# HakimNessah/th_rl

Measured on AMD Instinct MI355X. Metric: env-steps/sec, 2-agent PD x 1M parallel games, higher is better.
Workload: dtype f32

## Files before the change

### th_rl_amd/csrc/thrl_wave_kernel.h

```cpp
#pragma once
#include <type_traits>
#include <utility>
#include "thrl_kernels.h"
#include "thrl_wave_lut.h"

#ifndef THRL_ABLATE
#define THRL_ABLATE 0
#endif

namespace thrl {

constexpr int kAblate = THRL_ABLATE;

typedef unsigned int v2u __attribute__((ext_vector_type(2)));

__device__ __forceinline__ v2u pack_halves(unsigned a, unsigned b) {
    return __builtin_amdgcn_permlane32_swap(a, b, false, false);
}

__device__ __forceinline__ unsigned lds_addr(const void* p) {
    return (unsigned)(uintptr_t)(__attribute__((address_space(3))) const void*)p;
}
template <typename QT>
__device__ __forceinline__ QT lds_load(unsigned addr) {
    typedef __attribute__((address_space(3))) QT lds_t;
    return *(const lds_t*)(uintptr_t)addr;
}
template <typename QT>
__device__ __forceinline__ void lds_store(unsigned addr, QT v) {
    typedef __attribute__((address_space(3))) QT lds_t;
    *(lds_t*)(uintptr_t)addr = v;
}

__device__ __forceinline__ void lds_inc(unsigned addr) {
    typedef unsigned __attribute__((may_alias)) u32_alias;
    typedef __attribute__((address_space(3))) u32_alias lds_u32;
    __hip_atomic_fetch_add((lds_u32*)(uintptr_t)addr, 1u, __ATOMIC_RELAXED, __HIP_MEMORY_SCOPE_WAVEFRONT);
}
__device__ __forceinline__ void lds_zero8(unsigned addr) {
    typedef unsigned long long __attribute__((may_alias)) u64_alias;
    typedef __attribute__((address_space(3))) u64_alias lds_u64;
    *(lds_u64*)(uintptr_t)addr = 0ull;
}

__device__ __forceinline__ unsigned bperm(unsigned byte_sel, unsigned v) {
    return (unsigned)__builtin_amdgcn_ds_bpermute((int)byte_sel, (int)v);
}

template <int CTRL>
__device__ __forceinline__ double dpp_mov64(double v) {
    const int lo = __double2loint(v), hi = __double2hiint(v);
    return __hiloint2double(__builtin_amdgcn_update_dpp(hi, hi, CTRL, 0xF, 0xF, false),
                            __builtin_amdgcn_update_dpp(lo, lo, CTRL, 0xF, 0xF, false));
}
template <int CTRL>
__device__ __forceinline__ uint32_t dpp_mov32(uint32_t v) {
    return (uint32_t)__builtin_amdgcn_update_dpp((int)v, (int)v, CTRL, 0xF, 0xF, false);
}

__device__ __forceinline__ float group8_allmax(float v) {
    asm("s_nop 1\n\t"
        "v_max_f32_dpp %0, %0, %0 quad_perm:[1,0,3,2] row_mask:0xf bank_mask:0xf\n\t"
        "s_nop 1\n\t"
        "v_max_f32_dpp %0, %0, %0 quad_perm:[2,3,0,1] row_mask:0xf bank_mask:0xf\n\t"
        "s_nop 1\n\t"
        "v_max_f32_dpp %0, %0, %0 row_half_mirror row_mask:0xf bank_mask:0xf"
        : "+v"(v));
    return v;
}
__device__ __forceinline__ double group8_allmax(double v) {
    v = fmax(v, dpp_mov64<0xB1>(v));
    v = fmax(v, dpp_mov64<0x4E>(v));
    v = fmax(v, dpp_mov64<0x141>(v));
    return v;
}
__device__ __forceinline__ void store_where(unsigned long long mask, unsigned addr, float v) {
    unsigned long long save;
    asm volatile("s_mov_b64 %0, exec\n\ts_mov_b64 exec, %1\n\tds_write_b32 %2, %3\n\ts_mov_b64 exec, %0"
                 : "=&s"(save) : "s"(mask), "v"(addr), "v"(v) : "memory");
}
__device__ __forceinline__ void store_where(unsigned long long mask, unsigned addr, double v) {
    unsigned long long save;
    asm volatile("s_mov_b64 %0, exec\n\ts_mov_b64 exec, %1\n\tds_write_b64 %2, %3\n\ts_mov_b64 exec, %0"
                 : "=&s"(save) : "s"(mask), "v"(addr), "v"(v) : "memory");
}
template <int IMM>
__device__ __forceinline__ void store_key(unsigned key, unsigned want, unsigned addr, float v) {
    if constexpr (IMM >= 0)
        asm volatile("v_cmpx_eq_u32 vcc, %0, %1\n\tds_write_b32 %2, %3\n\ts_mov_b64 exec, -1"
                     :: "n"(IMM), "v"(key), "v"(addr), "v"(v) : "memory", "vcc");
    else
        asm volatile("v_cmpx_eq_u32 vcc, %0, %1\n\tds_write_b32 %2, %3\n\ts_mov_b64 exec, -1"
                     :: "s"(want), "v"(key), "v"(addr), "v"(v) : "memory", "vcc");
}
template <int IMM>
__device__ __forceinline__ void store_key(unsigned key, unsigned want, unsigned addr, double v) {
    if constexpr (IMM >= 0)
        asm volatile("v_cmpx_eq_u32 vcc, %0, %1\n\tds_write_b64 %2, %3\n\ts_mov_b64 exec, -1"
                     :: "n"(IMM), "v"(key), "v"(addr), "v"(v) : "memory", "vcc");
    else
        asm volatile("v_cmpx_eq_u32 vcc, %0, %1\n\tds_write_b64 %2, %3\n\ts_mov_b64 exec, -1"
                     :: "s"(want), "v"(key), "v"(addr), "v"(v) : "memory", "vcc");
}
constexpr unsigned kKeyShift = 25;
constexpr unsigned kKeyNone = 0x7Fu;
__device__ __forceinline__ float dpp_ror8(float v) { return __builtin_bit_cast(float, dpp_mov32<0x128>(__builtin_bit_cast(uint32_t, v))); }
__device__ __forceinline__ double dpp_ror8(double v) { return dpp_mov64<0x128>(v); }
__device__ __forceinline__ float max_of(float a, float b) { return fmaxf(a, b); }
__device__ __forceinline__ double max_of(double a, double b);
__device__ __forceinline__ float half32_allmax(float v) {
    v = group8_allmax(v);
    v = fmaxf(v, __builtin_bit_cast(float, dpp_mov32<0x140>(__builtin_bit_cast(uint32_t, v))));
    unsigned a = __builtin_bit_cast(unsigned, v), b = a;
    asm("" : "+v"(b));
    const v2u r = __builtin_amdgcn_permlane16_swap(a, b, false, false);
    const unsigned rx = r.x, ry = r.y;
    return fmaxf(__builtin_bit_cast(float, rx), __builtin_bit_cast(float, ry));
}
__device__ __forceinline__ double half32_allmax(double v) {
    v = group8_allmax(v);
    v = fmax(v, dpp_mov64<0x140>(v));
    unsigned lo = (unsigned)__double2loint(v), hi = (unsigned)__double2hiint(v);
    unsigned lo2 = lo, hi2 = hi;
    asm("" : "+v"(lo2), "+v"(hi2));
    const v2u rl = __builtin_amdgcn_permlane16_swap(lo, lo2, false, false);
    const v2u rh = __builtin_amdgcn_permlane16_swap(hi, hi2, false, false);
    const unsigned rlx = rl.x, rly = rl.y, rhx = rh.x, rhy = rh.y;
    return fmax(__hiloint2double((int)rhx, (int)rlx), __hiloint2double((int)rhy, (int)rly));
}
__device__ __forceinline__ double max_of(double a, double b) { return fmax(a, b); }

__device__ __forceinline__ double wave_sum4(double q0, double q1, double q2, double q3, int lane) {
    const bool odd = lane & 1;
    const double k0 = odd ? q1 : q0, k1 = odd ? q3 : q2;
    const double s0 = odd ? q0 : q1, s1 = odd ? q2 : q3;
    const double a0 = k0 + dpp_mov64<0xB1>(s0);
    const double a1 = k1 + dpp_mov64<0xB1>(s1);
    const bool b1 = lane & 2;
    const double kk = b1 ? a1 : a0, ss = b1 ? a0 : a1;
    double v = kk + dpp_mov64<0x4E>(ss);
    v = v + dpp_mov64<0x124>(v);
    v = v + dpp_mov64<0x128>(v);
    {
        unsigned lo = (unsigned)__double2loint(v), hi = (unsigned)__double2hiint(v);
        unsigned lo2 = lo, hi2 = hi;
        asm("" : "+v"(lo2), "+v"(hi2));
        const v2u rl = __builtin_amdgcn_permlane16_swap(lo, lo2, false, false);
        const v2u rh = __builtin_amdgcn_permlane16_swap(hi, hi2, false, false);
        const unsigned rlx = rl.x, rly = rl.y, rhx = rh.x, rhy = rh.y;
        v = __hiloint2double((int)rhx, (int)rlx) + __hiloint2double((int)rhy, (int)rly);
    }
    {
        unsigned lo = (unsigned)__double2loint(v), hi = (unsigned)__double2hiint(v);
        unsigned lo2 = lo, hi2 = hi;
        asm("" : "+v"(lo2), "+v"(hi2));
        const v2u rl = __builtin_amdgcn_permlane32_swap(lo, lo2, false, false);
        const v2u rh = __builtin_amdgcn_permlane32_swap(hi, hi2, false, false);
        const unsigned rlx = rl.x, rly = rl.y, rhx = rh.x, rhy = rh.y;
        v = __hiloint2double((int)rhx, (int)rlx) + __hiloint2double((int)rhy, (int)rly);
    }
    return v;
}

template <int CTRL>
__device__ __forceinline__ uint32_t dpp_src(uint32_t v) {
    return (uint32_t)__builtin_amdgcn_update_dpp(0, (int)v, CTRL, 0xF, 0xF, true);
}

__device__ __forceinline__ float max3_f32(float a, float b, float c) {
    float r;
    asm("v_max3_f32 %0, %1, %2, %3" : "=v"(r) : "v"(a), "v"(b), "v"(c));
    return r;
}
__device__ __forceinline__ uint32_t argmax21_first(unsigned row) {
    float g[7];
#pragma unroll
    for (int k = 0; k < 7; k++)
        g[k] = max3_f32(lds_load<float>(row + 12u * k), lds_load<float>(row + 12u * k + 4u), lds_load<float>(row + 12u * k + 8u));
    const float m = max3_f32(max3_f32(g[0], g[1], g[2]), max3_f32(g[3], g[4], g[5]), g[6]);
    uint32_t c3 = 18u;
#pragma unroll
    for (int k = 5; k >= 0; k--) c3 = (g[k] == m) ? (uint32_t)(3 * k) : c3;
    const unsigned ad = row + 4u * c3;
    const float va = lds_load<float>(ad), vb = lds_load<float>(ad + 4u);
    uint32_t pos = (vb == m) ? 1u : 2u;
    pos = (va == m) ? 0u : pos;
    const float v0 = lds_load<float>(row);
    return (v0 != v0) ? 0u : c3 + pos;
}

__device__ __forceinline__ uint32_t readlane_u(uint32_t v, int lane) {
    return (uint32_t)__builtin_amdgcn_readlane((int)v, lane);
}

__device__ __forceinline__ uint32_t writelane_u(uint32_t old, uint32_t val, int lane) {
    asm("s_mov_b32 m0, %2\n\ts_nop 0\n\tv_writelane_b32 %0, %1, m0" : "+v"(old) : "s"(val), "s"(lane));
    return old;
}

__device__ __forceinline__ uint32_t halves_sum(uint32_t x) {
    uint32_t y;
    asm("v_add_u32_sdwa %0, %1, %1 dst_sel:DWORD dst_unused:UNUSED_PAD src0_sel:WORD_0 src1_sel:WORD_1" : "=v"(y) : "v"(x));
    return y;
}

template <int T0>
__device__ __forceinline__ void chain_group(uint32_t& sq, int& s, uint32_t n0, uint32_t n1, uint32_t n2, uint32_t n3) {
    int s1, s2, s3, s4, pk;
    asm volatile(
        "s_nop 3\n\t"
        "v_readlane_b32 %1, %7, %6\n\t"
        "s_pack_ll_b32_b16 %5, %6, %1\n\t"
        "v_writelane_b32 %0, %5, %11\n\t"
        "s_nop 1\n\t"
        "v_readlane_b32 %2, %8, %1\n\t"
        "s_nop 3\n\t"
        "v_readlane_b32 %3, %9, %2\n\t"
        "s_pack_ll_b32_b16 %5, %2, %3\n\t"
        "v_writelane_b32 %0, %5, %12\n\t"
        "s_nop 1\n\t"
        "v_readlane_b32 %4, %10, %3"
        : "+v"(sq), "=&s"(s1), "=&s"(s2), "=&s"(s3), "=&s"(s4), "=&s"(pk)
        : "s"(s), "v"(n0), "v"(n1), "v"(n2), "v"(n3), "n"(T0), "n"(T0 + 2)
        : "scc");
    s = s4;
}

template <int T0>
__device__ __forceinline__ void chain_group_greedy(uint32_t& sq, int& s, uint32_t g1, uint32_t g2, uint32_t g3, uint32_t g4) {
    int s1, s2, s3, s4, pk;
    asm volatile(
        "s_nop 3\n\t"
        "v_readlane_b32 %1, %7, %6\n\t"
        "v_readlane_b32 %2, %8, %6\n\t"
        "v_readlane_b32 %3, %9, %6\n\t"
        "v_readlane_b32 %4, %10, %6\n\t"
        "s_pack_ll_b32_b16 %5, %6, %1\n\t"
        "v_writelane_b32 %0, %5, %11\n\t"
        "s_pack_ll_b32_b16 %5, %2, %3\n\t"
        "v_writelane_b32 %0, %5, %12"
        : "+v"(sq), "=&s"(s1), "=&s"(s2), "=&s"(s3), "=&s"(s4), "=&s"(pk)
        : "s"(s), "v"(g1), "v"(g2), "v"(g3), "v"(g4), "n"(T0), "n"(T0 + 2)
        : "scc");
    s = s4;
}

template <bool ON> struct GreedyTables {
    __device__ __forceinline__ void build(unsigned) {}
    template <int T0> __device__ __forceinline__ void chain(uint32_t&, int&) const {}
};
template <> struct GreedyTables<true> {
    uint32_t g1, g2, g3, g4;
    __device__ __forceinline__ void build(unsigned lut_addr) {
        g1 = (uint32_t)lds_load<unsigned short>(lut_addr);
        g2 = bperm((g1 & 63u) << 2, g1);
        g3 = bperm((g2 & 63u) << 2, g1);
        g4 = bperm((g2 & 63u) << 2, g2);
    }
    template <int T0> __device__ __forceinline__ void chain(uint32_t& sq, int& s) const { chain_group_greedy<T0>(sq, s, g1, g2, g3, g4); }
};

template <int NRSEG>
__device__ __forceinline__ uint32_t read_row(const uint32_t (&r)[NRSEG], int s) {
    uint32_t v = readlane_u(r[0], s & 63);
    if (NRSEG > 1) {
        const uint32_t h = readlane_u(r[NRSEG - 1], s & 63);
        if (s >= 64) v = h;
    }
    return v;
}
template <int NRSEG>
__device__ __forceinline__ uint32_t gather_row(const uint32_t (&r)[NRSEG], uint32_t row) {
    uint32_t v = bperm((row & 63u) << 2, r[0]);
    if (NRSEG > 1) {
        const uint32_t h = bperm((row & 63u) << 2, r[NRSEG - 1]);
        if (row >= 64u) v = h;
    }
    return v;
}

template <typename QT> struct BlockOps;
template <> struct BlockOps<float> {
    unsigned c1;
    __device__ __forceinline__ void permute(unsigned sel) { c1 = bperm(sel, c1); }
    __device__ __forceinline__ void keep() const { asm volatile("" :: "v"(c1)); }
    __device__ __forceinline__ float value(float nm, float alpha_gamma, float, float) const {
        return __fmaf_rn(alpha_gamma, nm, __builtin_bit_cast(float, c1));
    }
};
template <> struct BlockOps<double> {
    unsigned r_lo, r_hi, t4_lo, t4_hi;
    __device__ __forceinline__ void keep() const { asm volatile("" :: "v"(r_lo), "v"(r_hi), "v"(t4_lo), "v"(t4_hi)); }
    __device__ __forceinline__ void permute(unsigned sel) {
        r_lo = bperm(sel, r_lo); r_hi = bperm(sel, r_hi); t4_lo = bperm(sel, t4_lo); t4_hi = bperm(sel, t4_hi);
    }
// ... 164 lines not shown
    const unsigned colb = (unsigned)min(lane & 31, A - 1) * (unsigned)sizeof(QT);
#pragma unroll
    for (int j = 0; j < P; j++) {
        const unsigned sel = (unsigned)((lane & 32) + j) << 2;
        ops[j] = ops0;
        ops[j].permute(sel);
        cell[j] = bperm(sel, woq_x);
        const unsigned ad = tabh + ((W[j] >> 16) & 0xFFu) * row_bytes + colb;
        const QT v = lds_load<QT>(ad);
        cur[j] = lds_load<QT>(cell[j]);
        rest[j] = half32_allmax(ad == cell[j] ? -(QT)INFINITY : v);
    }
    int t = 0;
    for (; t + P <= nseg; t += P) {
#pragma unroll
        for (int j = 0; j < P; j++) cur[j] = ops[j].value(max_of(rest[(j + 1) % P], cur[(j + 1) % P]), alpha_gamma, alpha, gamma);
    }
#pragma unroll
    for (int j = 0; j < P; j++)
        if (t + j < nseg) cur[j] = ops[j].value(max_of(rest[(j + 1) % P], cur[(j + 1) % P]), alpha_gamma, alpha, gamma);
    if ((lane & 31) == 0) {
#pragma unroll
        for (int j = 0; j < P; j++) lds_store<QT>(cell[j], cur[j]);
    }
}

__device__ __forceinline__ uint32_t pack16(uint32_t lo, uint32_t hi) {
    typedef unsigned short v2h __attribute__((ext_vector_type(2)));
    return __builtin_bit_cast(uint32_t, v2h{(unsigned short)lo, (unsigned short)hi});
}
template <int L>
__device__ __forceinline__ uint32_t writelane_imm(uint32_t old, uint32_t val) {
    asm("v_writelane_b32 %0, %1, %2" : "+v"(old) : "s"(val), "n"(L));
    return old;
}
template <int T0>
__device__ __forceinline__ void chain_group_affine(uint32_t& sq, uint32_t& sc, uint32_t Tq) {
    const uint32_t s1 = readlane_u(Tq, (int)sc) & 0xFFu;
    const uint32_t s2 = (readlane_u(Tq, (int)s1) >> 8) & 0xFFu;
    const uint32_t s3 = (readlane_u(Tq, (int)s2) >> 16) & 0xFFu;
    const uint32_t s4 = readlane_u(Tq, (int)s3) >> 24;
    const uint32_t w = pack16(sc, s2) | (pack16(s1, s3) << 8);
    sq = writelane_imm<T0>(sq, w);
    sc = s4;
}
__device__ __forceinline__ uint32_t play_affine(int seg, int n, int lane, uint32_t rw, uint32_t G0q, uint32_t G1q, unsigned mk_addr,
                                                int c, int m0, int m1, int& s) {
    const int s_entry = __builtin_amdgcn_readfirstlane(s);
    {
        const uint32_t kb = (uint32_t)c - ((rw & 1u) ? ((rw >> 8) & 0xFFu) * (uint32_t)m0 : 0u)
                                        - ((rw & 2u) ? ((rw >> 16) & 0xFFu) * (uint32_t)m1 : 0u);
        const unsigned ad = mk_addr + 16u * (unsigned)(lane >> 2) + (unsigned)(lane & 3);
        lds_store<unsigned char>(ad, (rw & 1u) ? (unsigned char)0 : (unsigned char)0xFF);
        lds_store<unsigned char>(ad + 4u, (rw & 2u) ? (unsigned char)0 : (unsigned char)0xFF);
        lds_store<unsigned char>(ad + 8u, (unsigned char)kb);
        __builtin_amdgcn_wave_barrier();
    }
    struct Q4 { v2u lo, hi; };
    auto loadq = [&](int g) {
        Q4 q;
        q.lo = lds_load<v2u>(mk_addr + 16u * (unsigned)g);
        q.hi = lds_load<v2u>(mk_addr + 16u * (unsigned)g + 8u);
        return q;
    };
    auto make = [&](const Q4& q) {
        asm volatile("" :: "v"(q.hi.y));
        return q.hi.x - (G0q & q.lo.x) - (G1q & q.lo.y);
    };
    uint32_t sq = 0u, sq_tail = 0u;
    uint32_t sc = (uint32_t)s_entry & 0xFFu;
    auto chain4 = [&](auto t0c, const int nn, const uint32_t Tq) {
        constexpr int t0 = decltype(t0c)::value;
        __builtin_amdgcn_sched_barrier(0);
        if (t0 + 4 <= nn) chain_group_affine<t0>(sq, sc, Tq);
        else {
#pragma unroll
            for (int j = 0; j < 4; j++) {
                if (t0 + j < nn) {
                    sq_tail = writelane_u(sq_tail, sc * 0x101u, t0 + j);
                    sc = (readlane_u(Tq, (int)sc) >> (8 * j)) & 0xFFu;
                }
            }
        }
        __builtin_amdgcn_sched_barrier(0);
    };
    Q4 qa = loadq(0), qb = loadq(1);
    uint32_t Ta = make(qa), Tb = 0u;
#define THRL_PLAYA2(G, N_)                                                                   \
    if ((G) * 4 < (N_)) {                                                                    \
        if ((G) * 4 + 8 < (N_)) qa = loadq((G) + 2 < 15 ? (G) + 2 : 15);                     \
        chain4(std::integral_constant<int, (G) * 4>(), (N_), Ta);                            \
        if ((G) * 4 + 4 < (N_)) {                                                            \
            Tb = make(qb);                                                                   \
            if ((G) * 4 + 12 < (N_)) qb = loadq((G) + 3 < 15 ? (G) + 3 : 15);                \
            chain4(std::integral_constant<int, (G) * 4 + 4>(), (N_), Tb);                    \
            if ((G) * 4 + 8 < (N_)) Ta = make(qa);                                           \
        }                                                                                    \
    }
#define THRL_PLAYA16(N_)                                                                     \
    THRL_PLAYA2(0, N_) THRL_PLAYA2(2, N_) THRL_PLAYA2(4, N_) THRL_PLAYA2(6, N_)              \
    THRL_PLAYA2(8, N_) THRL_PLAYA2(10, N_) THRL_PLAYA2(12, N_) THRL_PLAYA2(14, N_)
    if (n == 64) { THRL_PLAYA16(64) } else if (n == 36) { THRL_PLAYA16(36) } else { THRL_PLAYA16(n) }
#undef THRL_PLAYA16
#undef THRL_PLAYA2
    s = (int)(sc * 0x101u);
    uint32_t qd;
    asm("s_nop 1\n\tv_mov_b32_dpp %0, %1 quad_perm:[0,0,0,0] row_mask:0xf bank_mask:0xf" : "=v"(qd) : "v"(sq));
    const uint32_t un = ((qd >> (8u * (unsigned)(lane & 3))) & 0xFFu) * 0x101u;
    uint32_t out = lane < (n & ~3) ? un : sq_tail;
    if (seg == 0) out = writelane_imm<0>(out, (uint32_t)s_entry);
    return out;
}

template <typename QT, int NSEG, int NRSEG, bool NOISE, bool SWEEP, bool CYCLE, bool GREEDY = false, bool LOG = false, bool AFFINE = false>
__global__ void __launch_bounds__(1024)
__attribute__((amdgpu_waves_per_eu(sizeof(QT) == 8 ? 3 : (NOISE ? 4 : (NSEG <= 2 ? 5 : 4)))))
k_wave_episodes(const WaveArgs a) {
    extern __shared__ __attribute__((aligned(16))) unsigned char smem[];
    static_assert(!AFFINE || (sizeof(QT) == 4 && !NOISE && !SWEEP && !CYCLE && !GREEDY && NRSEG == 1 && kAblate == 0),
                  "closed-form play tables: plain float32 variants with one row register");
    constexpr bool kUnrollReplay = NSEG <= 2 && !(NOISE && sizeof(QT) == 8);
    const int lane = threadIdx.x & 63;
    const int wib = __builtin_amdgcn_readfirstlane((int)(threadIdx.x >> 6));
    const int A = a.A, W = a.win_rows, Tenv = a.T, epk = CYCLE ? a.epk : 1, T = a.T * epk, lo = a.row_lo;
    const int replay_from = CYCLE ? a.replay_from : 0;
    const WaveLut L = wave_lut_layout(A);

    {
        const uint32_t* src = reinterpret_cast<const uint32_t*>(a.lut_ns);
        uint32_t* dst = reinterpret_cast<uint32_t*>(smem);
        for (int k = threadIdx.x; k < (a.lut_bytes >> 2); k += blockDim.x) dst[k] = src[k];
    }
    __syncthreads();
    const unsigned lut_ns_lds = lds_addr(smem + L.ns_off);
    const double* lut_aq = reinterpret_cast<const double*>(smem + L.aq_off);
    const double* lut_sct = reinterpret_cast<const double*>(smem + L.sct_off);

    QT* tab0 = reinterpret_cast<QT*>(smem + a.lut_bytes + (size_t)wib * a.game_lds_bytes);
    QT* tab1 = tab0 + (W + 2) * A;
    const int half = lane >> 5;
    const unsigned tab0_off = lds_addr(tab0);
    const unsigned tab1_off = lds_addr(tab1);
    const int kk = (lane >> 3) & 3, jj = lane & 7;
    const unsigned perm_sel = (unsigned)((lane & 32) + 4 * jj + kk) << 2;
    const unsigned my_step = (unsigned)(4 * jj + kk);
    const unsigned row_shift = (unsigned)(7 * kk);
    const unsigned row_bytes = (unsigned)A * (unsigned)sizeof(QT);
    const int rdn = A < 3 ? 2 : (A <= 24 ? 3 : 4);
    const unsigned rd_base = (half ? tab1_off : tab0_off) + (unsigned)sizeof(QT) * (unsigned)min(rdn * jj, A - rdn);
    constexpr bool kLdsMK = sizeof(QT) == 4 && !NOISE && !GREEDY && NRSEG == 1 && !(kAblate & 6);
    const unsigned mk_addr = tab0_off + 2u * (unsigned)((W + 2) * A) * (unsigned)sizeof(QT);
    constexpr bool kArgmax21 = sizeof(QT) == 4;
    constexpr bool kMaskSched = !NOISE && !GREEDY;

    const AgentParams& p0 = a.ag[0];
    const AgentParams& p1 = a.ag[1];
    const double inv_T_den = (double)Tenv;

    long long acc = 0, acc_hi = 0;
    const double log_scale = (lane & 2) ? a.log_scale[1] : a.log_scale[0];
    const int wave_gid = blockIdx.x * a.waves_per_block + wib;

    int g_claim = 0;
    if (lane == 0) g_claim = atomicAdd(a.next_game, 1);
    for (;;) {
        const int g = __builtin_amdgcn_readfirstlane(g_claim);
        if (g >= a.G) break;
        if (lane == 0) g_claim = atomicAdd(a.next_game, 1);
        const uint64_t gid = a.game_offset + (uint64_t)g;
        QT* __restrict__ q0 = reinterpret_cast<QT*>(a.q) + (int64_t)g * a.stride + p0.table_off;
        QT* __restrict__ q1 = reinterpret_cast<QT*>(a.q) + (int64_t)g * a.stride + p1.table_off;
        const double price0 = a.state[g];

        QT gamma_h = half ? HP<QT>::gamma(p1) : HP<QT>::gamma(p0);
        QT alpha_h = half ? HP<QT>::alpha(p1) : HP<QT>::alpha(p0);
        QT oma0 = HP<QT>::one_minus_alpha(p0), oma1 = HP<QT>::one_minus_alpha(p1);
        if (SWEEP && a.sw_gamma) gamma_h = HP<QT>::from_double(a.sw_gamma[(size_t)half * a.G + g]);
        if (SWEEP && a.sw_alpha) {
            alpha_h = HP<QT>::from_double(a.sw_alpha[(size_t)half * a.G + g]);
            oma0 = HP<QT>::from_double(__dsub_rn(1.0, a.sw_alpha[g]));
            oma1 = HP<QT>::from_double(__dsub_rn(1.0, a.sw_alpha[(size_t)a.G + g]));
        }
        double epsg0 = 0.0, epsg1 = 0.0;
        const bool sw_eps_on = SWEEP && a.sw_eps != nullptr;
        if (sw_eps_on) { epsg0 = a.sw_eps[g]; epsg1 = a.sw_eps[(size_t)a.G + g]; }
        const QT ag_h = HP<QT>::product(alpha_h, gamma_h);
        const double eend0 = (SWEEP && a.sw_eps_end) ? a.sw_eps_end[g] : p0.eps_end;
        const double eend1 = (SWEEP && a.sw_eps_end) ? a.sw_eps_end[(size_t)a.G + g] : p1.eps_end;
        const double estep0 = (SWEEP && a.sw_eps_step) ? a.sw_eps_step[g] : p0.eps_step;
        const double estep1 = (SWEEP && a.sw_eps_step) ? a.sw_eps_step[(size_t)a.G + g] : p1.eps_step;
        const double noise_prob_g = (SWEEP && a.sw_noise_prob) ? a.sw_noise_prob[g] : a.env.noise_prob;

        {
            const QT* s0 = q0 + lo * A;
            const QT* s1 = q1 + lo * A;
            const int n = W * A;
            for (int k0 = 0; k0 < n; k0 += 512) {
                QT v0[8], v1[8];
#pragma unroll
                for (int j = 0; j < 8; j++) {
                    const int k = min(k0 + j * 64 + lane, n - 1);
                    v0[j] = s0[k]; v1[j] = s1[k];
                }
#pragma unroll
                for (int j = 0; j < 8; j++) {
                    const int k = k0 + j * 64 + lane;
                    if (k < n) { tab0[k] = v0[j]; tab1[k] = v1[j]; }
                }
            }
        }
        int sp = __builtin_amdgcn_readfirstlane(encode32(price0, p0));
        int st = __builtin_amdgcn_readfirstlane(encode64(price0, p0));
        sp = min(max(sp, 0), a.rows - 1);
        st = min(max(st, 0), a.rows - 1);
        int spill0 = -1, spill1 = -1, sp_l, st_l;
        if (sp >= lo && sp < lo + W) sp_l = sp - lo; else { spill0 = sp; sp_l = W; }
        if (st == sp) st_l = sp_l;
        else if (st >= lo && st < lo + W) st_l = st - lo;
        else { spill1 = st; st_l = W + 1; }

        {
            if (spill0 >= 0 && lane < A) {
                tab0[W * A + lane] = q0[spill0 * A + lane];
                tab1[W * A + lane] = q1[spill0 * A + lane];
            }
            if (spill1 >= 0 && lane < A) {
                tab0[(W + 1) * A + lane] = q0[spill1 * A + lane];
                tab1[(W + 1) * A + lane] = q1[spill1 * A + lane];
            }
        }
        __builtin_amdgcn_wave_barrier();

        int s = sp_l | (st_l << 8);
        double last_price = price0;
        for (int e = 0; e < a.n_episodes; e += epk) {
            const uint32_t eg = (uint32_t)(a.first_episode + (uint64_t)e);

            uint32_t AM[NRSEG], R[NRSEG];
            uint32_t G0q = 0u, G1q = 0u;
#pragma unroll
            for (int k = 0; k < NRSEG; k++) {
                const int row = min(lane + 64 * k, W + 1);
                const QT* r0 = tab0 + row * A;
                const QT* r1 = tab1 + row * A;
                QT b0 = r0[0], b1 = r1[0];
                uint32_t i0 = 0, i1 = 0;
                if (kAblate & 16) {
                } else if (kArgmax21 && A == 21) {
                    i0 = argmax21_first(tab0_off + (unsigned)row * 84u);
                    i1 = argmax21_first(tab1_off + (unsigned)row * 84u);
                } else if (A == 21) {
#pragma unroll
                    for (int j = 1; j < 21; j++) {
                        const QT v0 = r0[j], v1 = r1[j];
                        if (v0 > b0) { b0 = v0; i0 = j; }
                        if (v1 > b1) { b1 = v1; i1 = j; }
                    }
                } else {
#pragma unroll 4
                    for (int j = 1; j < A; j++) {
                        const QT v0 = r0[j], v1 = r1[j];
                        if (v0 > b0) { b0 = v0; i0 = j; }
                        if (v1 > b1) { b1 = v1; i1 = j; }
                    }
                }
                if (kAblate & 16) { i0 = (uint32_t)(lane * 5) % (uint32_t)A; i1 = (uint32_t)(lane * 3) % (uint32_t)A; }
                AM[k] = i0 | (i1 << 8);
                R[k] = (i0 * (uint32_t)A * 2u) | (i1 << 17);
                if constexpr (AFFINE) {
                    G0q = i0 * ((uint32_t)a.aff_m0 * 0x01010101u);
                    G1q = i1 * ((uint32_t)a.aff_m1 * 0x01010101u);
                }
            }
            GreedyTables<GREEDY && NRSEG == 1> gt;
            gt.build(halves_sum(R[0]) + lut_ns_lds);

            uint32_t seq[NSEG], rwv[NSEG];
            unsigned explored_segs = 0u;
            double nav[NSEG];
#pragma unroll
            for (int seg = 0; seg < NSEG; seg++) {
                int n = min(64, T - seg * 64);
                asm volatile("" : "+s"(n));
                uint32_t rw;
                nav[seg] = 0.0;
                const int tcl = min(seg * 64 + lane, T - 1);
                const int ep = epk == 1 ? 0 : tcl / Tenv;
                const uint32_t st_in_ep = (uint32_t)(tcl - ep * Tenv);
                double eps0, eps1;
                if (sw_eps_on) { eps0 = epsg0; eps1 = epsg1; }
                else if (epk == 1) { eps0 = a.eps[e][0]; eps1 = a.eps[e][1]; }
                else { eps0 = a.eps[e + ep][0]; eps1 = a.eps[e + ep][1]; }
                if (a.inj_u) {
                    const int tt = tcl;
                    const size_t k = (((size_t)e * Tenv + tt) * 2) * (size_t)a.G + (size_t)g;
                    const uint32_t ex0 = a.inj_u[k] < eps0 ? 1u : 0u;
                    const uint32_t ex1 = a.inj_u[k + a.G] < eps1 ? 2u : 0u;
                    const uint32_t c0 = min((uint32_t)(uint8_t)a.inj_choice[k], (uint32_t)(A - 1));
                    const uint32_t c1 = min((uint32_t)(uint8_t)a.inj_choice[k + a.G], (uint32_t)(A - 1));
                    rw = ex0 | ex1 | (c0 << 8) | (c1 << 16);
                } else if (kAblate & 8) {
                    const uint32_t h = (uint32_t)(lane * 2654435761u) ^ eg;
                    rw = (h & 3u) | (((h >> 4) % (uint32_t)A) << 8) | (((h >> 12) % (uint32_t)A) << 16);
                } else {
                    uint32_t seed_lo = (uint32_t)a.seed, seed_hi = (uint32_t)(a.seed >> 32);
                    asm volatile("" : "+s"(seed_lo), "+s"(seed_hi));
                    const uint64_t seed_here = ((uint64_t)seed_hi << 32) | seed_lo;
                    const u32x4 x = draw_lanes(seed_here, gid, eg + (uint32_t)ep, st_in_ep, 0u);
                    const uint32_t ex0 = u01_32(x.x) < eps0 ? 1u : 0u;
                    const uint32_t ex1 = u01_32(x.z) < eps1 ? 2u : 0u;
                    rw = ex0 | ex1 | (__umulhi(x.y, (uint32_t)A) << 8) | (__umulhi(x.w, (uint32_t)A) << 16);
                }
                if (NOISE) {
                    double nu, na;
// ... 206 lines not shown
                    }
                }
                const long long vq = __double2ll_rn(__dmul_rn(v, log_scale));
                if ((lane >> 2) == (epi & 15)) { if (epi < 16) acc += vq; else acc_hi += vq; }
            };
#pragma unroll
            for (int seg = 0; seg < NSEG; seg++) {
                const int tt = seg * 64 + lane;
                const bool valid = tt < T;
                const uint32_t a0 = act[seg] & 0xFFu, a1 = (act[seg] >> 8) & 0xFFu;
                const double aq0 = lut_aq[a0], aq1 = lut_aq[A + a1];
                const double a_eff = (NOISE && (rwv[seg] & 4u)) ? nav[seg] : a.env.a;
                double price = __dsub_rn(a_eff, __dmul_rn(a.env.b, __dadd_rn(aq0, aq1)));
                if (!(price > 0.0)) price = 0.0;
                const double r0d = __dmul_rn(price, aq0);
                const double r1d = __dmul_rn(price, aq1);
                if (seg == NSEG - 1) {
                    const int ll = T - 1 - seg * 64;
                    last_price = __hiloint2double(__builtin_amdgcn_readlane(__double2hiint(price), ll),
                                                  __builtin_amdgcn_readlane(__double2loint(price), ll));
                }
                if (epk == 1) {
                    if (valid) {
                        lr0 += r0d; lr1 += r1d;
                        la0 += lut_sct[a0]; la1 += lut_sct[A + a1];
                    }
                } else {
                    const int ep_l = min(tt, T - 1) / Tenv;
                    const int j0 = (seg * 64) / Tenv, j1 = (min(T, seg * 64 + 64) - 1) / Tenv;
                    const double s0 = lut_sct[a0], s1 = lut_sct[A + a1];
                    for (int j = j0; j <= j1; j++) {
                        const bool m = valid && ep_l == j;
                        log_into(e + j, m ? r0d : 0.0, m ? r1d : 0.0, m ? s0 : 0.0, m ? s1 : 0.0, j * Tenv >= seg * 64);
                    }
                }
                const bool trains = valid && tt >= replay_from;
                if (a.counter && !(kAblate & 32))
                    a.tlog[(((size_t)wave_gid * kWaveMaxEpisodes + e) * NSEG + seg) * 64 + lane] =
                        trains ? cwv[seg] : 0xFFFFFFFFu;

                uint32_t P, cutq;
                bool any_fixed;
                const unsigned long long pairs = __ballot(CYCLE ? (valid && tt > replay_from) : valid);
                const uint32_t quad0 = (uint32_t)lane & 60u;
                if (kAblate & 128) { P = (act[seg] >> 24) * 0x204081u; any_fixed = false; cutq = 0u; }
                else if constexpr (kMaskSched) {
                    const uint32_t w = act[seg];
                    const uint32_t d = (w >> 24) ^ ((w >> 16) & 0xFFu);
                    uint32_t x0 = w ^ dpp_src<0x00>(w), x1 = w ^ dpp_src<0x55>(w), x2 = w ^ dpp_src<0xAA>(w);
                    asm("" : "+v"(x0), "+v"(x1), "+v"(x2));
                    auto hz = [&](uint32_t x) -> unsigned long long {
                        const uint32_t xr = (x >> 16) & 0xFFu;
                        return __ballot((((x & 0xFFu) * ((x >> 8) & 0xFFu)) | xr) == 0u) | __ballot(xr == d);
                    };
                    const unsigned long long H0 = hz(x0), H1 = hz(x1), H2 = hz(x2);
                    const unsigned long long M = 0x1111111111111111ull;
                    const unsigned long long C1 = (H0 >> 1) & M;
                    const unsigned long long C2 = ((H1 >> 2) | ((H0 >> 2) & ~C1)) & M;
                    const unsigned long long C3 = ((H2 >> 3) | (((H1 >> 3) | ((H0 >> 3) & ~C1)) & ~C2)) & M;
                    const unsigned long long F = (__ballot((x0 | x1 | x2) == 0u) >> 3) & __ballot(d == 0u) & M;
                    const unsigned long long sched = (C1 & (pairs >> 1)) | ((C2 & (pairs >> 2)) << 1) | ((C3 & (pairs >> 3)) << 2) | (F << 3);
                    any_fixed = F != 0ull;
                    uint32_t rows = (w >> 24) << (7u * ((uint32_t)lane & 3u));
                    rows |= dpp_src<0xB1>(rows);
                    rows |= dpp_src<0x4E>(rows);
                    cutq = (uint32_t)(sched >> quad0);
                    P = (cutq << 28) | rows;
                } else {
                    const uint32_t w = act[seg];
                    const uint32_t b0 = dpp_mov32<0x00>(w), b1 = dpp_mov32<0x55>(w), b2 = dpp_mov32<0xAA>(w),
                                   b3 = dpp_mov32<0xFF>(w);
                    const uint32_t qp = (uint32_t)lane & 3u;
                    auto hz = [&](uint32_t bi, uint32_t i) -> uint32_t {
                        const bool raw = (w >> 24) == ((bi >> 16) & 0xFFu);
                        const bool waw = ((w >> 16) & 0xFFu) == ((bi >> 16) & 0xFFu) &&
                                         ((w & 0xFFu) == (bi & 0xFFu) || ((w >> 8) & 0xFFu) == ((bi >> 8) & 0xFFu));
                        return (qp > i && (raw || waw)) ? 1u : 0u;
                    };
                    const uint32_t hzw = hz(b0, 0u) | (hz(b1, 1u) << 1) | (hz(b2, 2u) << 2);
                    const uint32_t h1 = dpp_mov32<0x55>(hzw), h2 = dpp_mov32<0xAA>(hzw), h3 = dpp_mov32<0xFF>(hzw);
                    const uint32_t c1 = h1 & 1u;
                    const uint32_t c2 = ((h2 >> 1) & 1u) | ((c1 ^ 1u) & h2 & 1u);
                    const uint32_t c3 = ((h3 >> 2) & 1u) | ((c2 ^ 1u) & (((h3 >> 1) & 1u) | ((c1 ^ 1u) & h3 & 1u)));
                    bool quad_quiet = true;
                    if (NOISE) quad_quiet = ((__ballot((rwv[seg] & 4u) != 0u) >> (lane & 60)) & 0xFull) == 0ull;
                    const uint32_t same4 = ((quad_quiet && b0 == b1 && b1 == b2 && b2 == b3 && (b0 >> 24) == ((b0 >> 16) & 0xFFu)) ||
                                            (GREEDY && b0 == b2 && b1 == b3 && (b0 >> 24) == ((b1 >> 16) & 0xFFu) &&
                                             (b1 >> 24) == ((b0 >> 16) & 0xFFu) && (b0 >> 24) != (b1 >> 24))) ? 1u : 0u;
                    cutq = (c1 | (c2 << 1) | (c3 << 2)) & ((uint32_t)(pairs >> quad0) >> 1);
                    P = (b0 >> 24) | ((b1 >> 24) << 7) | ((b2 >> 24) << 14) | ((b3 >> 24) << 21) |
                        (cutq << 28) | (same4 << 31);
                    any_fixed = __ballot((P >> 31) != 0u) != 0ull;
                }

                const uint32_t pass_no = (uint32_t)__builtin_popcount(cutq & ((1u << ((uint32_t)lane & 3u)) - 1u));
                const uint32_t key_base = tab0_off + ((trains ? (quad0 & 28u) + pass_no : kKeyNone) << kKeyShift);
                const v2u woq = pack_halves(key_base + (cwv[seg] & 0xFFFFu) * kCellScale, key_base + (cwv[seg] >> 16) * kCellScale);

                bool seg_done = false;
                if (GREEDY && !(kAblate & 257) && !((explored_segs >> seg) & 1u)) {
                    const int nseg = min(64, T - seg * 64);
                    const uint32_t w = act[seg];
                    const uint32_t w1 = dpp_mov32<0x138>(w), w2 = dpp_mov32<0x138>(w1);
                    const uint32_t w3 = dpp_mov32<0x138>(w2), w4 = dpp_mov32<0x138>(w3);
                    const bool in_seg = lane < nseg;
                    const int period = __ballot(in_seg && lane >= 1 && w != w1) == 0ull ? 1
                                     : __ballot(in_seg && lane >= 2 && w != w2) == 0ull ? 2
                                     : __ballot(in_seg && lane >= 3 && w != w3) == 0ull ? 3
                                     : __ballot(in_seg && lane >= 4 && w != w4) == 0ull ? 4 : 0;
                    if (period > 0 && nseg >= period) {
                        uint32_t W[4];
#pragma unroll
                        for (int j = 0; j < 4; j++) W[j] = readlane_u(w, j);
                        bool ok = true;
#pragma unroll
                        for (int j = 0; j < 4; j++)
                            if (j < period) {
                                const uint32_t nxt_row = (W[(j + 1 < period) ? j + 1 : 0] >> 16) & 0xFFu;
                                ok = ok && (W[j] >> 24) == nxt_row;
#pragma unroll
                                for (int i = 0; i < j; i++) ok = ok && ((W[i] >> 16) & 0xFFu) != ((W[j] >> 16) & 0xFFu);
                            }
                        if (ok) {
                            seg_done = true;
                            const BlockOps<QT> ops0 = make_ops(snap[seg], 0, r0d, r1d, alpha_h);
                            const unsigned tabh = half ? tab1_off : tab0_off;
                            const unsigned wo_step = woq.x & ((1u << kKeyShift) - 1u);
                            if (period == 1) cyclic_segment<QT, 1>(ops0, wo_step, W, nseg, lane, tabh, A, row_bytes, ag_h, alpha_h, gamma_h);
                            else if (period == 2) cyclic_segment<QT, 2>(ops0, wo_step, W, nseg, lane, tabh, A, row_bytes, ag_h, alpha_h, gamma_h);
                            else if (period == 3) cyclic_segment<QT, 3>(ops0, wo_step, W, nseg, lane, tabh, A, row_bytes, ag_h, alpha_h, gamma_h);
                            else cyclic_segment<QT, 4>(ops0, wo_step, W, nseg, lane, tabh, A, row_bytes, ag_h, alpha_h, gamma_h);
                            __builtin_amdgcn_wave_barrier();
                        }
                    }
                }
#pragma unroll
                for (int k = 0; k < 2; k++) {
                    if (GREEDY && seg_done) break;
                    int nsub = __builtin_amdgcn_readfirstlane(min(32, T - seg * 64 - k * 32));
                    asm volatile("" : "+s"(nsub));
                    if (nsub <= 0) break;
                    BlockOps<QT> ops = make_ops(snap[seg], k, r0d, r1d, alpha_h);
                    ops.permute(perm_sel);
                    const unsigned wo = bperm(perm_sel, k ? woq.y : woq.x);
#define THRL_REPLAY(RDN_, FP_) replay_block<QT, RDN_, FP_, kUnrollReplay && RDN_ == 3, GREEDY>(P, k * 32, nsub, ops, wo, rd_base, row_shift, my_step, row_bytes, \
                                                          ag_h, alpha_h, gamma_h, half != 0, seg * 64 + k * 32, replay_from)
                    if (A > 24)      { if (any_fixed) THRL_REPLAY(4, true); else THRL_REPLAY(4, false); }
                    else if (A >= 3) { if (any_fixed) THRL_REPLAY(3, true); else THRL_REPLAY(3, false); }
                    else             { if (any_fixed) THRL_REPLAY(2, true); else THRL_REPLAY(2, false); }
#undef THRL_REPLAY
                }
            }

            if (epk == 1) log_into(e, lr0, lr1, la0, la1, true);
            if (SWEEP) {
                epsg0 = __dadd_rn(eend0, __dmul_rn(__dsub_rn(epsg0, eend0), estep0));
                epsg1 = __dadd_rn(eend1, __dmul_rn(__dsub_rn(epsg1, eend1), estep1));
            }
        }

        {
            QT* d0 = q0 + lo * A;
            QT* d1 = q1 + lo * A;
            const int n = W * A;
            for (int k = lane; k < n; k += 64) { d0[k] = tab0[k]; d1[k] = tab1[k]; }
            if (spill0 >= 0 && lane < A) {
                q0[spill0 * A + lane] = tab0[W * A + lane];
                q1[spill0 * A + lane] = tab1[W * A + lane];
            }
            if (spill1 >= 0 && lane < A) {
                q0[spill1 * A + lane] = tab0[(W + 1) * A + lane];
                q1[spill1 * A + lane] = tab1[(W + 1) * A + lane];
            }
            if (lane == 0 && a.n_episodes > 0) a.state[g] = last_price;
            if (lane == 0 && sw_eps_on) { a.sw_eps[g] = epsg0; a.sw_eps[(size_t)a.G + g] = epsg1; }
        }
        __builtin_amdgcn_wave_barrier();

        if (a.counter && !(kAblate & 32)) {
            const int cells = (W + 2) * A;
            typedef unsigned __attribute__((may_alias)) hist_u32;
            hist_u32* hist = reinterpret_cast<hist_u32*>(tab0);
            __builtin_amdgcn_fence(__ATOMIC_SEQ_CST, "wavefront");
            for (int k = lane; k < cells; k += 64) lds_zero8(tab0_off + 8u * (unsigned)k);
            __builtin_amdgcn_wave_barrier();
            const int n_cycles = a.n_episodes / epk;
            for (int c0 = 0; c0 < n_cycles; c0 += 4) {
                unsigned w[4][NSEG];
#pragma unroll
                for (int j = 0; j < 4; j++)
#pragma unroll
                    for (int seg = 0; seg < NSEG; seg++)
                        w[j][seg] = __hip_atomic_load(
                            &a.tlog[(((size_t)wave_gid * kWaveMaxEpisodes + min(c0 + j, n_cycles - 1) * epk) * NSEG + seg) * 64 + lane],
                            __ATOMIC_RELAXED, __HIP_MEMORY_SCOPE_AGENT);
#pragma unroll
                for (int j = 0; j < 4; j++)
#pragma unroll
                    for (int seg = 0; seg < NSEG; seg++) {
                        const unsigned ww = w[j][seg];
                        if (c0 + j < n_cycles && ww != 0xFFFFFFFFu) {
                            lds_inc(tab0_off + (ww & 0xFFFFu));
                            lds_inc(tab0_off + (ww >> 16));
                        }
                    }
            }
            __builtin_amdgcn_wave_barrier();
            int32_t* cw0 = a.counter + (int64_t)g * a.stride + p0.table_off;
            int32_t* cw1 = a.counter + (int64_t)g * a.stride + p1.table_off;
            const int nwin = W * A;
            auto add = [](int32_t* p, unsigned n) {
                if (n) __hip_atomic_fetch_add(p, (int32_t)n, __ATOMIC_RELAXED, __HIP_MEMORY_SCOPE_AGENT);
            };
            for (int k = lane; k < nwin; k += 64) {
                add(cw0 + lo * A + k, hist[k]);
                add(cw1 + lo * A + k, hist[cells + k]);
            }
            if (lane < 2 * A) {
                const int which = lane >= A, col = lane - which * A;
                const int grow_ = which ? spill1 : spill0;
                if (grow_ >= 0) {
                    add(cw0 + grow_ * A + col, hist[nwin + lane]);
                    add(cw1 + grow_ * A + col, hist[cells + nwin + lane]);
                }
            }
            __builtin_amdgcn_fence(__ATOMIC_SEQ_CST, "wavefront");
            __builtin_amdgcn_wave_barrier();
        }
    }
    a.partial[(size_t)wave_gid * 128 + lane] = acc;
    a.partial[(size_t)wave_gid * 128 + 64 + lane] = acc_hi;
}

template <typename QT, int NSEG, int NRSEG, bool NOISE, bool SWEEP, bool CYCLE, bool GREEDY, bool LOG, bool AFFINE = false>
static int launch_wave_t(const WaveArgs& a, int grid, int block, size_t lds, hipStream_t s) {
    auto kern = k_wave_episodes<QT, NSEG, NRSEG, NOISE, SWEEP, CYCLE, GREEDY, LOG, AFFINE>;
    if (lds > 64 * 1024) {
        const hipError_t e = hipFuncSetAttribute(reinterpret_cast<const void*>(kern),
                                                 hipFuncAttributeMaxDynamicSharedMemorySize, (int)lds);
        if (e != hipSuccess) return (int)e;
    }
    hipLaunchKernelGGL(kern, dim3(grid), dim3(block), lds, s, a);
    return (int)hipGetLastError();
}

template <typename QT, bool NOISE, bool SWEEP, bool CYCLE, bool GREEDY, bool LOG>
static int launch_wave_nl(const WaveArgs& a, int grid, int block, size_t lds, hipStream_t s) {
    const int nseg = (a.T * a.epk + 63) / 64;
    const int nrseg = (a.win_rows + 2 + 63) / 64;
    if (nrseg == 1) {
        switch (nseg) {
            case 1: return launch_wave_t<QT, 1, 1, NOISE, SWEEP, CYCLE, GREEDY, LOG>(a, grid, block, lds, s);
            case 2: return launch_wave_t<QT, 2, 1, NOISE, SWEEP, CYCLE, GREEDY, LOG>(a, grid, block, lds, s);
            case 3: return launch_wave_t<QT, 3, 1, NOISE, SWEEP, CYCLE, GREEDY, LOG>(a, grid, block, lds, s);
            case 4: return launch_wave_t<QT, 4, 1, NOISE, SWEEP, CYCLE, GREEDY, LOG>(a, grid, block, lds, s);
        }
    } else if (nrseg == 2) {
        switch (nseg) {
            case 1: return launch_wave_t<QT, 1, 2, NOISE, SWEEP, CYCLE, GREEDY, LOG>(a, grid, block, lds, s);
            case 2: return launch_wave_t<QT, 2, 2, NOISE, SWEEP, CYCLE, GREEDY, LOG>(a, grid, block, lds, s);
            case 3: return launch_wave_t<QT, 3, 2, NOISE, SWEEP, CYCLE, GREEDY, LOG>(a, grid, block, lds, s);
            case 4: return launch_wave_t<QT, 4, 2, NOISE, SWEEP, CYCLE, GREEDY, LOG>(a, grid, block, lds, s);
        }
    }
    return -1;
}

template <typename QT, bool NOISE, bool SWEEP, bool CYCLE, bool GREEDY = false>
static int launch_wave_n(const WaveArgs& a, int grid, int block, size_t lds, hipStream_t s) {
    if (a.game_reward_log || a.game_action_log) return launch_wave_nl<QT, NOISE, SWEEP, CYCLE, GREEDY, true>(a, grid, block, lds, s);
    return launch_wave_nl<QT, NOISE, SWEEP, CYCLE, GREEDY, false>(a, grid, block, lds, s);
}

}
```

Before: 47.84 billion.

## Park per-episode log sums in global memory and finish them after the episode loop

When neither LOG nor CYCLE is enabled, each episode's reward/action sums are reduced with wave_sum4 and written with a masked global store into a per-wave scratch buffer. They are no longer accumulated through log_into inside the episode loop. After the game finishes, the parked values are reloaded, scaled, quantized and added to the accumulators, overlapping with the histogram pass when counting is on. The goal is to move the divide, multiply and conversion work off the hot per-episode path. The change also adds a dpp_src64 helper that uses bound_ctrl DPP for the row-shift adds, and it relies on a.partial having room for kWaveMaxEpisodes*4 entries per wave.

```diff
diff --git a/th_rl_amd/csrc/thrl_wave_kernel.h b/th_rl_amd/csrc/thrl_wave_kernel.h
--- a/th_rl_amd/csrc/thrl_wave_kernel.h
+++ b/th_rl_amd/csrc/thrl_wave_kernel.h
@@ -83,6 +83,10 @@
     unsigned long long save;
     asm volatile("s_mov_b64 %0, exec\n\ts_mov_b64 exec, %1\n\tds_write_b64 %2, %3\n\ts_mov_b64 exec, %0"
                  : "=&s"(save) : "s"(mask), "v"(addr), "v"(v) : "memory");
+}
+__device__ __forceinline__ void store_lanes(unsigned long long mask, long long* base, unsigned off, double v) {
+    asm volatile("s_mov_b64 exec, %0\n\tglobal_store_dwordx2 %1, %2, %3\n\ts_mov_b64 exec, -1"
+                 :: "s"(mask), "v"(off), "v"(v), "s"(base) : "memory");
 }
 template <int IMM>
 __device__ __forceinline__ void store_key(unsigned key, unsigned want, unsigned addr, float v) {
@@ -130,6 +134,13 @@
 }
 __device__ __forceinline__ double max_of(double a, double b) { return fmax(a, b); }
 
+template <int CTRL>
+__device__ __forceinline__ double dpp_src64(double v) {
+    const int lo = __double2loint(v), hi = __double2hiint(v);
+    return __hiloint2double(__builtin_amdgcn_update_dpp(0, hi, CTRL, 0xF, 0xF, true),
+                            __builtin_amdgcn_update_dpp(0, lo, CTRL, 0xF, 0xF, true));
+}
+
 __device__ __forceinline__ double wave_sum4(double q0, double q1, double q2, double q3, int lane) {
     const bool odd = lane & 1;
     const double k0 = odd ? q1 : q0, k1 = odd ? q3 : q2;
@@ -139,8 +150,8 @@
     const bool b1 = lane & 2;
     const double kk = b1 ? a1 : a0, ss = b1 ? a0 : a1;
     double v = kk + dpp_mov64<0x4E>(ss);
-    v = v + dpp_mov64<0x124>(v);
-    v = v + dpp_mov64<0x128>(v);
+    v = v + dpp_src64<0x124>(v);
+    v = v + dpp_src64<0x128>(v);
     {
         unsigned lo = (unsigned)__double2loint(v), hi = (unsigned)__double2hiint(v);
         unsigned lo2 = lo, hi2 = hi;
@@ -611,6 +622,7 @@
     const unsigned mk_addr = tab0_off + 2u * (unsigned)((W + 2) * A) * (unsigned)sizeof(QT);
     constexpr bool kArgmax21 = sizeof(QT) == 4;
     constexpr bool kMaskSched = !NOISE && !GREEDY;
+    constexpr bool kParkLogs = !LOG && !CYCLE;
 
     const AgentParams& p0 = a.ag[0];
     const AgentParams& p1 = a.ag[1];
@@ -619,6 +631,19 @@
     long long acc = 0, acc_hi = 0;
     const double log_scale = (lane & 2) ? a.log_scale[1] : a.log_scale[0];
     const int wave_gid = blockIdx.x * a.waves_per_block + wib;
+    auto load_parked = [&](int pass) {
+        return __hip_atomic_load(&a.partial[(size_t)wave_gid * 128 + 64 * pass + lane], __ATOMIC_RELAXED, __HIP_MEMORY_SCOPE_AGENT);
+    };
+    auto finish_parked = [&](long long p0w, long long p1w) {
+#pragma unroll
+        for (int pass = 0; pass < 2; pass++) {
+            if (pass == 1 && a.n_episodes <= 16) break;
+            double v = __longlong_as_double(pass ? p1w : p0w);
+            if ((lane & 3) < 2) v = __ddiv_rn(v, inv_T_den);
+            const long long vq = __double2ll_rn(__dmul_rn(v, log_scale));
+            if (16 * pass + (lane >> 2) < a.n_episodes) { if (pass) acc_hi += vq; else acc += vq; }
+        }
+    };
 
     int g_claim = 0;
     if (lane == 0) g_claim = atomicAdd(a.next_game, 1);
@@ -1131,7 +1156,10 @@
                 }
             }
 
-            if (epk == 1) log_into(e, lr0, lr1, la0, la1, true);
+            if constexpr (kParkLogs) {
+                const double v = (kAblate & 64) ? lr0 + lr1 + la0 + la1 : wave_sum4(lr0, lr1, la0, la1, lane);
+                store_lanes(0xFull << (4 * (e & 3)), a.partial + ((size_t)wave_gid * kWaveMaxEpisodes + e) * 4, ((unsigned)lane & 3u) << 3, v);
+            } else if (epk == 1) log_into(e, lr0, lr1, la0, la1, true);
             if (SWEEP) {
                 epsg0 = __dadd_rn(eend0, __dmul_rn(__dsub_rn(epsg0, eend0), estep0));
                 epsg1 = __dadd_rn(eend1, __dmul_rn(__dsub_rn(epsg1, eend1), estep1));
@@ -1156,7 +1184,14 @@
         }
         __builtin_amdgcn_wave_barrier();
 
-        if (a.counter && !(kAblate & 32)) {
+        const bool counting = a.counter && !(kAblate & 32);
+        if constexpr (kParkLogs) {
+            if (!counting && a.n_episodes > 0) {
+                const long long p0w = load_parked(0), p1w = load_parked(1);
+                finish_parked(p0w, p1w);
+            }
+        }
+        if (counting) {
             const int cells = (W + 2) * A;
             typedef unsigned __attribute__((may_alias)) hist_u32;
             hist_u32* hist = reinterpret_cast<hist_u32*>(tab0);
@@ -1164,6 +1199,8 @@
             for (int k = lane; k < cells; k += 64) lds_zero8(tab0_off + 8u * (unsigned)k);
             __builtin_amdgcn_wave_barrier();
             const int n_cycles = a.n_episodes / epk;
+            long long p0w = 0, p1w = 0;
+            if constexpr (kParkLogs) { p0w = load_parked(0); p1w = load_parked(1); }
             for (int c0 = 0; c0 < n_cycles; c0 += 4) {
                 unsigned w[4][NSEG];
 #pragma unroll
@@ -1184,6 +1221,7 @@
                         }
                     }
             }
+            if constexpr (kParkLogs) finish_parked(p0w, p1w);
             __builtin_amdgcn_wave_barrier();
             int32_t* cw0 = a.counter + (int64_t)g * a.stride + p0.table_off;
             int32_t* cw1 = a.counter + (int64_t)g * a.stride + p1.table_off;
```

Measured after the change: 48.67 billion (median of 6 runs). 1.7% higher.
